# SludgePhD/Compeg

Hardware: AMD Instinct MI355X
Metric: Mpixels/s decoded (4K 4:2:2 restart-interval baseline JPEG -> RGBA8 in HBM) (higher is better)
Workload: dtype u32 bit-reader / i16 levels / f32 IDCT / u8 RGBA

## Files before the change

compeg_amd/csrc/kernels.hip:

```cpp
#include <hip/hip_runtime.h>

#include <algorithm>
#include <atomic>
#include <cstdio>
#include <cstdlib>

#include "kernels_body.h"
#include "coop_body.h"
#include "walk_body.h"
#include "kernels.h"
#include "lab.h"

namespace compeg {

struct DeviceLimits {
    uint32_t cus, lds_bytes;
};
static DeviceLimits device_limits()
{
    static std::atomic<uint64_t> known[64];
    int dev = 0;
    const bool indexed = hipGetDevice(&dev) == hipSuccess && dev >= 0 && dev < 64;
    if (indexed) {
        const uint64_t k = known[dev].load(std::memory_order_relaxed);
// ... 63 lines not shown
    const ImageDesc &d = descs[blockIdx.y];
    const uint32_t first_interval = blockIdx.x * blockDim.x;
    if (first_interval >= d.total_intervals)
        return;

    uint16_t *l1 = reinterpret_cast<uint16_t *>(smem);
    uint16_t *l2 = l1 + kL1Entries;
    const uint32_t wave_area = align16(window_words * 4u) + kWave * kDuSlotBytes;
    uint8_t *wave_base = smem + align16((kL1Entries + l2_in_lds) * 2u);

    stage_luts(d, l1, l2, l2_in_lds, threadIdx.x, blockDim.x);

    const uint32_t wave = threadIdx.x / kWave, lane = threadIdx.x % kWave;
    uint32_t *win = reinterpret_cast<uint32_t *>(wave_base + wave * wave_area);
    const uint32_t wave_first = first_interval + wave * kWave;
    uint32_t win_base = 0, win_len = 0;
    if (wave_first < d.total_intervals) {
        wave_window(d, wave_first, window_words, win_base, win_len);
        stage_window(d, win, win_base, win_len, lane);
    }
    __syncthreads();

    if (wave_first >= d.total_intervals)
        return;

    HuffShared s;
    s.l1 = l1;
    s.l2 = l2;
    s.l2_staged = umin(l2_in_lds, d.fast_off + 2u * kFastEntries);
    s.win = win;
    s.win_base = win_base;
    s.win_len = win_len;
    s.du_slots = reinterpret_cast<uint8_t *>(win) + align16(window_words * 4u);
    entropy_wave_to_records<SAMPLES>(d, s, wave_first + lane, lane);
}

__global__ void __launch_bounds__(1024)
entropy_kernel(const ImageDesc *__restrict__ descs, uint32_t l2_in_lds, uint32_t window_words)
{
    entropy_kernel_body<false>(descs, l2_in_lds, window_words);
}

__global__ void __launch_bounds__(768)
entropy_samples_kernel(const ImageDesc *__restrict__ descs, uint32_t l2_in_lds, uint32_t window_words)
{
    entropy_kernel_body<true>(descs, l2_in_lds, window_words);
}

struct WindowAhead {
    const ImageDesc *descs;
    uint32_t image;
    bool any;
    uint32_t first;
    uint32_t window_words, lane;
    uint32_t *win;
    uint32_t raw_base, raw_end, base, len, sink;
    uint32_t *queue;
    uint32_t next, drawn, stride, units, waves_per_image, group;

    __device__ __forceinline__ void at(uint32_t du, uint32_t du_total)
    {
        if (queue) {
            if (du == 0u && lane == 0u)
                drawn = atomicAdd(queue, 1u);
            if (du == 1u) {
                next = (stride + uint32_t(__builtin_amdgcn_readfirstlane(int(drawn)))) * group;
                any = next < units;
                if (any) {
                    image = uint32_t(__builtin_amdgcn_readfirstlane(int(next / waves_per_image)));
                    first = uint32_t(__builtin_amdgcn_readfirstlane(int((next % waves_per_image) * kWave)));
                }
            }
        }
        if (!any)
            return;
        const ImageDesc *dn = descs + image;
        if (du == (queue ? 1u : 0u))
            wave_window_fetch(*dn, first, raw_base, raw_end);
        if (du_total >= 8u && du == (du_total >= 10u ? du_total - 8u : 2u)) {
            uint32_t b, l;
            wave_window_from(*dn, raw_base, raw_end, window_words, b, l);
            const uint32_t have = dn->nwords > b ? umin(l, dn->nwords - b) : 0u;
            auto *words = CG_GLOBAL(const uint32_t, dn->words);
            for (uint32_t v = lane * 32u; v < have; v += kWave * 32u)
                sink ^= words[b + v];
        }
        if (du_total >= 8u && du == (du_total >= 10u ? du_total - 5u : 5u))
            asm volatile("" ::"v"(sink));
    }

    __device__ __forceinline__ void decoded(uint32_t du, uint32_t du_total)
    {
        if (!any || du + 1u != du_total)
            return;
        const ImageDesc *dn = descs + image;
        uint32_t b, l;
        wave_window_from(*dn, raw_base, raw_end, window_words, b, l);
        base = uint32_t(__builtin_amdgcn_readfirstlane(int(b)));
        len = uint32_t(__builtin_amdgcn_readfirstlane(int(l)));
        stage_window(*dn, win, base, len, lane);
        __builtin_amdgcn_fence(__ATOMIC_RELEASE, "wavefront");
        __builtin_amdgcn_wave_barrier();
    }
};

template <class LAYOUT, uint32_t GROUP>
__device__ __forceinline__ void fused_kernel_body(const ImageDesc *__restrict__ descs, uint32_t l2_in_lds, uint32_t window_words,
                                                  uint32_t waves_per_image, uint32_t images, uint32_t *queue)
{
    constexpr uint32_t group = GROUP;
    extern __shared__ __attribute__((aligned(16))) uint8_t smem[];
    const uint32_t wave = uint32_t(__builtin_amdgcn_readfirstlane(int(threadIdx.x / kWave))), lane = threadIdx.x % kWave;
    uint32_t image = blockIdx.y, wave_first = (blockIdx.x * (blockDim.x / kWave) + wave) * kWave;
    bool has_work = true;
    if (waves_per_image) {
        const uint32_t flat = (blockIdx.x * (blockDim.x / kWave) + wave) * (queue ? group : 1u);
        image = flat / waves_per_image;
        wave_first = (flat % waves_per_image) * kWave;
        has_work = image < images;
        image = has_work ? image : images - 1u;
    }
    image = uint32_t(__builtin_amdgcn_readfirstlane(int(image)));
    wave_first = uint32_t(__builtin_amdgcn_readfirstlane(int(wave_first)));
    if (!waves_per_image && blockIdx.x * blockDim.x >= descs[image].total_intervals)
        return;
    has_work = has_work && wave_first < descs[image].total_intervals;

    uint16_t *l1 = reinterpret_cast<uint16_t *>(smem);
    uint16_t *l2 = l1 + kL1Entries;
    const uint32_t wave_area = align16(window_words * 4u) + kWave * kDuSlotBytes;
    uint8_t *wave_base = smem + align16((kL1Entries + l2_in_lds) * 2u);
    uint32_t *win = reinterpret_cast<uint32_t *>(wave_base + wave * wave_area);
    uint8_t *slots = reinterpret_cast<uint8_t *>(win) + align16(window_words * 4u);

    uint32_t win_base = 0, win_len = 0;
    if (has_work)
        wave_window(descs[image], wave_first, window_words, win_base, win_len);
    stage_luts_and_window(descs[image], l1, l2, l2_in_lds, threadIdx.x, blockDim.x, win, win_base, win_len, lane);
    __syncthreads();

    if (!has_work)
        return;

    const uint32_t stride = gridDim.x * (blockDim.x / kWave), units = waves_per_image * images;
    const uint32_t per_draw = waves_per_image && queue ? group : 1u;
    uint32_t flat = (blockIdx.x * (blockDim.x / kWave) + wave) * per_draw;
    for (;;) {
        const ImageDesc &d = descs[image];
        HuffShared s;
        s.l1 = l1;
        s.l2 = l2;
        s.l2_staged = umin(l2_in_lds, d.fast_off + 2u * kFastEntries);
        s.win = win;
        s.win_base = win_base;
        s.win_len = win_len;
        s.du_slots = slots;
        const bool draw = waves_per_image && queue && flat % per_draw == per_draw - 1u;
        flat += waves_per_image && queue ? 1u : stride;
        WindowAhead ahead;
        ahead.descs = descs;
        ahead.queue = draw ? queue : nullptr;
        ahead.stride = stride;
        ahead.units = units;
        ahead.waves_per_image = waves_per_image;
        ahead.group = per_draw;
        ahead.next = ahead.drawn = 0u;
        ahead.any = waves_per_image && !draw && flat < units;
        ahead.image = ahead.first = 0u;
        if (ahead.any) {
            ahead.image = uint32_t(__builtin_amdgcn_readfirstlane(int(flat / waves_per_image)));
            ahead.first = uint32_t(__builtin_amdgcn_readfirstlane(int((flat % waves_per_image) * kWave)));
        }
        ahead.window_words = window_words;
        ahead.lane = lane;
        ahead.win = win;
        ahead.sink = 0u;
        LAYOUT::decode(d, s, wave_first + lane, lane, ahead);
        if (!ahead.any)
            break;
        if (draw)
            flat = ahead.next;
        image = ahead.image;
        wave_first = ahead.first;
        win_base = ahead.base;
        win_len = ahead.len;
    }
}

constexpr uint32_t kMcuQueueGroup = 4;

template <bool WIDE, bool RECORDS = false>
struct Wave422 {
    template <class AHEAD>
    static __device__ __forceinline__ void decode(const ImageDesc &d, const HuffShared &s, uint32_t interval, uint32_t lane, AHEAD &ahead)
    {
        decode_wave_fused_422<AHEAD, WIDE, RECORDS>(d, s, interval, lane, ahead);
    }
};
#if !defined(CG_FUSED_BOUNDS) || !defined(COMPEG_LAB)
#define CG_FUSED_BOUNDS 768
#endif
__global__ void __launch_bounds__(CG_FUSED_BOUNDS)
decode_fused_422_kernel(const ImageDesc *__restrict__ descs, uint32_t l2_in_lds, uint32_t window_words,
                        uint32_t waves_per_image, uint32_t images, uint32_t *queue)
{
    fused_kernel_body<Wave422<false>, 1>(descs, l2_in_lds, window_words, waves_per_image, images, queue);
}
__global__ void __launch_bounds__(768)
decode_fused_422_mcu_kernel(const ImageDesc *__restrict__ descs, uint32_t l2_in_lds, uint32_t window_words,
                            uint32_t waves_per_image, uint32_t images, uint32_t *queue)
{
    fused_kernel_body<Wave422<true>, kMcuQueueGroup>(descs, l2_in_lds, window_words, waves_per_image, images, queue);
}
__global__ void __launch_bounds__(768)
decode_fused_422_mcu_rec_kernel(const ImageDesc *__restrict__ descs, uint32_t l2_in_lds, uint32_t window_words,
                                uint32_t waves_per_image, uint32_t images, uint32_t *queue)
{
    fused_kernel_body<Wave422<true, true>, kMcuQueueGroup>(descs, l2_in_lds, window_words, waves_per_image, images, queue);
}
template <int HS, int VS, int MC>
__device__ __forceinline__ void fused_layout_kernel_body(const ImageDesc *__restrict__ descs, uint32_t l2_in_lds, uint32_t window_words)
{
    extern __shared__ __attribute__((aligned(16))) uint8_t smem[];
    const ImageDesc &d = descs[blockIdx.y];
    const uint32_t first_interval = blockIdx.x * blockDim.x;
    if (first_interval >= d.total_intervals)
        return;
    uint16_t *l1 = reinterpret_cast<uint16_t *>(smem);
    uint16_t *l2 = l1 + kL1Entries;
    const uint32_t wave_area = align16(window_words * 4u) + kWave * kDuSlotBytes;
    uint8_t *wave_base = smem + align16((kL1Entries + l2_in_lds) * 2u);
    const uint32_t wave = uint32_t(__builtin_amdgcn_readfirstlane(int(threadIdx.x / kWave))), lane = threadIdx.x % kWave;
    uint32_t *win = reinterpret_cast<uint32_t *>(wave_base + wave * wave_area);
    const uint32_t wave_first = first_interval + wave * kWave;
    uint32_t win_base = 0, win_len = 0;
    if (wave_first < d.total_intervals)
        wave_window(d, wave_first, window_words, win_base, win_len);
    stage_luts_and_window(d, l1, l2, l2_in_lds, threadIdx.x, blockDim.x, win, win_base, win_len, lane);
    __syncthreads();
    if (wave_first >= d.total_intervals)
        return;
// ... 1029 lines not shown
```

compeg_amd/csrc/kernels_body.h:

```cpp
#pragma once

#include <cstdint>
#include <cstring>

#include "device_types.h"

#if defined(__HIPCC__)
#define CG_DEV __device__ __forceinline__
#else
#define CG_DEV static inline
#endif

#if defined(__HIP_DEVICE_COMPILE__)
#define CG_GLOBAL(T, p) (reinterpret_cast<__attribute__((address_space(1))) T *>(reinterpret_cast<uintptr_t>(p)))
#define CG_PIN_SCALAR(x) asm volatile("" : "+s"(x))
#else
#define CG_GLOBAL(T, p) (p)
#define CG_PIN_SCALAR(x) (void)(x)
#endif

#ifndef CG_IDCT_PACKED
#define CG_IDCT_PACKED 1
#endif
#ifndef CG_PRIO_IDCT
#define CG_PRIO_IDCT 1
#endif
#ifndef CG_PRIO_ENTROPY
#define CG_PRIO_ENTROPY 0
#endif
#ifndef CG_PRIO_COMPOSITE
#define CG_PRIO_COMPOSITE 3
#endif
#ifndef CG_NT_STORES
#define CG_NT_STORES 1
#endif
#if !defined(COMPEG_LAB)
#undef CG_EXP
#endif
#ifndef CG_EXP
#define CG_EXP 0
#endif

namespace compeg {

struct alignas(16) Vec4u {
    uint32_t x, y, z, w;
};

template <bool STREAM>
CG_DEV void store_pixels(uint8_t *p, const Vec4u &v)
{
#if defined(COMPEG_LAB) && defined(CG_STORE_POLICY) && defined(__HIP_DEVICE_COMPILE__)
    if (STREAM) {
        typedef uint32_t u32x4 __attribute__((ext_vector_type(4)));
        const u32x4 val{v.x, v.y, v.z, v.w};
        asm volatile("global_store_dwordx4 %0, %1, off " CG_STORE_POLICY ::"v"(p), "v"(val) : "memory");
        return;
    }
#endif
#if CG_NT_STORES && defined(__HIP_DEVICE_COMPILE__)
    if (STREAM) {
        typedef uint32_t u32x4 __attribute__((ext_vector_type(4)));
        __builtin_nontemporal_store(
            u32x4{v.x, v.y, v.z, v.w},
            reinterpret_cast<__attribute__((address_space(1))) u32x4 *>(reinterpret_cast<uintptr_t>(p)));
        return;
    }
#endif
    *CG_GLOBAL(Vec4u, reinterpret_cast<Vec4u *>(p)) = v;
}


struct HuffShared {
    const uint16_t *l1;
    const uint16_t *l2;
    uint32_t l2_staged;
    const uint32_t *win;
    uint32_t win_base;
    uint32_t win_len;
    uint8_t *du_slots;
};

CG_DEV uint32_t bswap32(uint32_t w)
{
    return (w << 24) | ((w & 0xff00u) << 8) | ((w >> 8) & 0xff00u) | (w >> 24);
}

struct BitReader {
    uint32_t cur, nxt, left, next_word;
};

CG_DEV uint32_t fetch_word(const ImageDesc &d, const HuffShared &s, uint32_t idx)
{
    const uint32_t rel = idx - s.win_base;
    if (rel < s.win_len)
        return s.win[rel];
    return idx < d.nwords ? bswap32(CG_GLOBAL(const uint32_t, d.words)[idx]) : 0u;
}

CG_DEV void refill(BitReader &b, const ImageDesc &d, const HuffShared &s)
{
    if (b.left < 32u) {
        const uint32_t w = fetch_word(d, s, b.next_word);
        b.next_word += 1u;
        b.cur |= w >> (b.left & 31u);
        b.nxt = (w << 1) << ((31u - b.left) & 31u);
        b.left += 32u;
    }
}

CG_DEV void consume(BitReader &b, uint32_t n)
{
    b.cur = (b.cur << (n & 31u)) | ((b.nxt >> 1) >> ((31u - n) & 31u));
    b.nxt <<= (n & 31u);
    b.left -= n;
}

CG_DEV uint32_t peek(const BitReader &b, uint32_t n)
{
    return (b.cur >> 1) >> ((31u - n) & 31u);
}

CG_DEV int32_t huff_extend(int32_t v, uint32_t t)
// ... 947 lines not shown
    e.pred0 = comp == 0u ? p : p0;
    e.pred1 = comp == 1u ? p : p1;
    e.pred2 = comp == 2u ? p : p2;
    return int32_t(uint32_t(p) * d.dc_quant[comp]);
}


constexpr int kPxSlotWords = 17;

CG_DEV uint32_t ycbcr_to_rgba(uint32_t y_, uint32_t cb_, uint32_t cr_)
{
    const int32_t y = int32_t(y_), cb = int32_t(cb_) - 128, cr = int32_t(cr_) - 128;
    int32_t r = y + ((45 * cr) >> 5);
    int32_t g = y - ((11 * cb + 23 * cr) >> 5);
    int32_t b = y + ((113 * cb) >> 6);
    r = r < 0 ? 0 : (r > 255 ? 255 : r);
    g = g < 0 ? 0 : (g > 255 ? 255 : g);
    b = b < 0 ? 0 : (b > 255 ? 255 : b);
    return uint32_t(r) | uint32_t(g) << 8 | uint32_t(b) << 16 | 0xff000000u;
}

CG_DEV void composite_422(const ImageDesc &d, const uint32_t *px_slots, uint32_t first_mcu,
                          uint32_t total_mcus, uint32_t j)
{
    const uint32_t m = j >> 2, quarter = j & 3u;
    const uint32_t mcu = first_mcu + m;
    if (mcu >= total_mcus)
        return;
    const uint32_t mx = mcu % d.width_mcus, my = mcu / d.width_mcus;
    const uint32_t x0 = mx * 16u + quarter * 4u;
    if (x0 >= d.out_w)
        return;
    const uint32_t *ydu = px_slots + (m * 4u + (quarter >> 1)) * kPxSlotWords;
    const uint32_t *cbdu = px_slots + (m * 4u + 2u) * kPxSlotWords;
    const uint32_t *crdu = px_slots + (m * 4u + 3u) * kPxSlotWords;
    const uint32_t cshift = (quarter & 1u) * 16u;
#pragma unroll
    for (uint32_t row = 0; row < 8; row++) {
        const uint32_t y = my * 8u + row;
        if (y >= d.out_h)
            break;
        const uint32_t yw = ydu[row * 2u + (quarter & 1u)];
        const uint32_t cbw = cbdu[row * 2u + (quarter >> 1)] >> cshift;
        const uint32_t crw = crdu[row * 2u + (quarter >> 1)] >> cshift;
        Vec4u o;
        o.x = ycbcr_to_rgba(yw & 0xffu, cbw & 0xffu, crw & 0xffu);
        o.y = ycbcr_to_rgba((yw >> 8) & 0xffu, cbw & 0xffu, crw & 0xffu);
        o.z = ycbcr_to_rgba((yw >> 16) & 0xffu, (cbw >> 8) & 0xffu, (crw >> 8) & 0xffu);
        o.w = ycbcr_to_rgba(yw >> 24, (cbw >> 8) & 0xffu, (crw >> 8) & 0xffu);
        uint8_t *p = d.out + size_t(y) * d.out_pitch + size_t(x0) * 4u;
        if (x0 + 3u < d.out_w && (d.out_pitch & 15u) == 0u) {
            store_pixels<true>(p, o);
        } else {
            auto *q = CG_GLOBAL(uint32_t, reinterpret_cast<uint32_t *>(p));
            q[0] = o.x;
            if (x0 + 1u < d.out_w)
                q[1] = o.y;
            if (x0 + 2u < d.out_w)
                q[2] = o.z;
            if (x0 + 3u < d.out_w)
                q[3] = o.w;
        }
    }
}


CG_DEV uint32_t ycbcr_to_rgba(uint32_t y_, uint32_t cb_, uint32_t cr_);

CG_DEV Vec4u rgba_quad(uint32_t yw, uint32_t cb2, uint32_t cr2)
{
    Vec4u o;
#if defined(__HIP_DEVICE_COMPILE__)
    typedef short s2 __attribute__((ext_vector_type(2)));
    const s2 cb = __builtin_bit_cast(s2, __builtin_amdgcn_perm(0u, cb2, 0x0c010c00u));
    const s2 cr = __builtin_bit_cast(s2, __builtin_amdgcn_perm(0u, cr2, 0x0c010c00u));
    const s2 k45 = {45, 45}, k11 = {11, 11}, k23 = {23, 23}, k113 = {113, 113};
    const s2 b45 = {-5760, -5760}, b34 = {-4352, -4352}, b113 = {-14464, -14464};
    const s2 sh5 = {5, 5}, sh6 = {6, 6};
    const s2 rc = (cr * k45 + b45) >> sh5;
    const s2 gc = (cb * k11 + (cr * k23 + b34)) >> sh5;
    const s2 bc = (cb * k113 + b113) >> sh6;
    const s2 ya = __builtin_bit_cast(s2, yw & 0x00ff00ffu);
    const s2 yb = __builtin_bit_cast(s2, (yw >> 8) & 0x00ff00ffu);
    uint32_t ra, ga, ba, rb, gb, bb;
    asm("v_sat_pk_u8_i16 %0, %1" : "=v"(ra) : "v"(ya + rc));
    asm("v_sat_pk_u8_i16 %0, %1" : "=v"(ga) : "v"(ya - gc));
    asm("v_sat_pk_u8_i16 %0, %1" : "=v"(ba) : "v"(ya + bc));
    asm("v_sat_pk_u8_i16 %0, %1" : "=v"(rb) : "v"(yb + rc));
    asm("v_sat_pk_u8_i16 %0, %1" : "=v"(gb) : "v"(yb - gc));
    asm("v_sat_pk_u8_i16 %0, %1" : "=v"(bb) : "v"(yb + bc));
    const uint32_t rga = ga << 16 | ra, rgb = gb << 16 | rb;
    o.x = __builtin_amdgcn_perm(ba, rga, 0x0d040200u);
    o.z = __builtin_amdgcn_perm(ba, rga, 0x0d050301u);
    o.y = __builtin_amdgcn_perm(bb, rgb, 0x0d040200u);
    o.w = __builtin_amdgcn_perm(bb, rgb, 0x0d050301u);
#else
    o.x = ycbcr_to_rgba(yw & 0xffu, cb2 & 0xffu, cr2 & 0xffu);
    o.y = ycbcr_to_rgba((yw >> 8) & 0xffu, cb2 & 0xffu, cr2 & 0xffu);
    o.z = ycbcr_to_rgba((yw >> 16) & 0xffu, (cb2 >> 8) & 0xffu, (cr2 >> 8) & 0xffu);
    o.w = ycbcr_to_rgba(yw >> 24, (cb2 >> 8) & 0xffu, (cr2 >> 8) & 0xffu);
#endif
    return o;
}

CG_DEV Vec4u rgba_quad4(uint32_t yw, uint32_t cb4, uint32_t cr4)
{
    Vec4u o;
#if defined(__HIP_DEVICE_COMPILE__)
    typedef short s2 __attribute__((ext_vector_type(2)));
    const s2 k45 = {45, 45}, k11 = {11, 11}, k23 = {23, 23}, k113 = {113, 113};
    const s2 b45 = {-5760, -5760}, b34 = {-4352, -4352}, b113 = {-14464, -14464};
    const s2 sh5 = {5, 5}, sh6 = {6, 6};
    const s2 ya = __builtin_bit_cast(s2, yw & 0x00ff00ffu), yb = __builtin_bit_cast(s2, (yw >> 8) & 0x00ff00ffu);
    const s2 cba = __builtin_bit_cast(s2, cb4 & 0x00ff00ffu), cbb = __builtin_bit_cast(s2, (cb4 >> 8) & 0x00ff00ffu);
    const s2 cra = __builtin_bit_cast(s2, cr4 & 0x00ff00ffu), crb = __builtin_bit_cast(s2, (cr4 >> 8) & 0x00ff00ffu);
    uint32_t ra, ga, ba, rb, gb, bb;
    asm("v_sat_pk_u8_i16 %0, %1" : "=v"(ra) : "v"(ya + ((cra * k45 + b45) >> sh5)));
    asm("v_sat_pk_u8_i16 %0, %1" : "=v"(ga) : "v"(ya - ((cba * k11 + (cra * k23 + b34)) >> sh5)));
    asm("v_sat_pk_u8_i16 %0, %1" : "=v"(ba) : "v"(ya + ((cba * k113 + b113) >> sh6)));
    asm("v_sat_pk_u8_i16 %0, %1" : "=v"(rb) : "v"(yb + ((crb * k45 + b45) >> sh5)));
    asm("v_sat_pk_u8_i16 %0, %1" : "=v"(gb) : "v"(yb - ((cbb * k11 + (crb * k23 + b34)) >> sh5)));
    asm("v_sat_pk_u8_i16 %0, %1" : "=v"(bb) : "v"(yb + ((cbb * k113 + b113) >> sh6)));
    const uint32_t rga = ga << 16 | ra, rgb = gb << 16 | rb;
    o.x = __builtin_amdgcn_perm(ba, rga, 0x0d040200u);
    o.z = __builtin_amdgcn_perm(ba, rga, 0x0d050301u);
    o.y = __builtin_amdgcn_perm(bb, rgb, 0x0d040200u);
    o.w = __builtin_amdgcn_perm(bb, rgb, 0x0d050301u);
#else
    o.x = ycbcr_to_rgba(yw & 0xffu, cb4 & 0xffu, cr4 & 0xffu);
    o.y = ycbcr_to_rgba((yw >> 8) & 0xffu, (cb4 >> 8) & 0xffu, (cr4 >> 8) & 0xffu);
    o.z = ycbcr_to_rgba((yw >> 16) & 0xffu, (cb4 >> 16) & 0xffu, (cr4 >> 16) & 0xffu);
    o.w = ycbcr_to_rgba(yw >> 24, cb4 >> 24, cr4 >> 24);
#endif
    return o;
}


CG_DEV void composite_row_to_slot(const uint32_t (&px)[4][16], uint32_t row, uint8_t *slot)
{
    SlotVec *p = reinterpret_cast<SlotVec *>(slot);
#pragma unroll
    for (uint32_t q = 0; q < 4; q++) {
#if CG_EXP == 5
        p[q] = SlotVec{px[q >> 1][row * 2u + (q & 1u)], px[2][row * 2u + (q >> 1)], px[3][row * 2u + (q >> 1)], q};
#else
        const Vec4u o = rgba_quad(px[q >> 1][row * 2u + (q & 1u)], px[2][row * 2u + (q >> 1)] >> ((q & 1u) * 16u),
                                  px[3][row * 2u + (q >> 1)] >> ((q & 1u) * 16u));
        p[q] = SlotVec{o.x, o.y, o.z, o.w};
#endif
    }
}

CG_DEV void composite_row_from_quad(const ImageDesc &d, const uint8_t *wave_slots, uint32_t lane, uint32_t row,
                                    uint8_t *const (&bases)[4], uint32_t whole_mask)
{
    const uint32_t quad = lane & ~3u, piece = lane & 3u;
#pragma unroll
    for (uint32_t j = 0; j < 4; j++) {
        const SlotVec v = reinterpret_cast<const SlotVec *>(wave_slots + (quad + j) * kDuSlotBytes)[piece];
#if (CG_EXP == 9 || CG_EXP == 17 || CG_EXP == 18) && defined(__HIP_DEVICE_COMPILE__)
        asm volatile("" ::"v"(v.x), "v"(v.y), "v"(v.z), "v"(v.w));
        if (v.x == 0x12345678u && v.y == 0x9abcdef0u && bases[j] == nullptr)
#else
        if (whole_mask >> j & 1u)
#endif
        {
            store_pixels<true>(bases[j] + size_t(row) * d.out_pitch + piece * 16u, Vec4u{v.x, v.y, v.z, v.w});
        }
    }
}

CG_DEV uint32_t cut_rows_for_piece(uint32_t limits, uint32_t piece)
{
    uint32_t rows = 0u;
#pragma unroll
    for (uint32_t j = 0; j < 4; j++) {
        const uint32_t lim = (limits >> (8u * j)) & 0xffu;
        rows |= (piece < lim >> 5 ? lim & 31u : 0u) << (8u * j);
    }
    return rows;
}
CG_DEV uint32_t cut_row_inside(uint32_t rows, uint32_t row) { return (rows + 0x01010101u * (127u - row)) & 0x80808080u; }

CG_DEV void composite_row_from_wave(const ImageDesc &d, const uint8_t *wave_slots, uint32_t lane, uint32_t row,
                                    uint8_t *const (&bases)[4], uint32_t whole_mask)
{
    const uint32_t piece = lane & 3u, sub = lane >> 2;
#pragma unroll
    for (uint32_t t = 0; t < 4; t++) {
        const SlotVec v = reinterpret_cast<const SlotVec *>(wave_slots + (16u * t + sub) * kDuSlotBytes)[piece];
        if (whole_mask >> t & 1u)
            store_pixels<true>(bases[t] + size_t(row) * d.out_pitch + piece * 16u, Vec4u{v.x, v.y, v.z, v.w});
    }
}

CG_DEV void composite_edge_mcu(const ImageDesc &d, const uint32_t (&px)[4][16], uint32_t mx, uint32_t my)
{
    const uint32_t x0 = mx * 16u, y0 = my * 8u;
    uint8_t *base = d.out + size_t(y0) * d.out_pitch + size_t(x0) * 4u;
#pragma unroll 1
    for (uint32_t row = 0; row < 8; row++) {
        if (y0 + row >= d.out_h)
            break;
#pragma unroll 1
        for (uint32_t q = 0; q < 4; q++) {
            const uint32_t w = row * 2u + (q & 1u), c = row * 2u + (q >> 1);
            uint32_t yw = 0, cbw = 0, crw = 0;
#pragma unroll
            for (uint32_t i = 0; i < 16; i++) {
                yw = (i == w) ? ((q >> 1) ? px[1][i] : px[0][i]) : yw;
                cbw = (i == c) ? px[2][i] : cbw;
                crw = (i == c) ? px[3][i] : crw;
            }
            const Vec4u o = rgba_quad(yw, cbw >> ((q & 1u) * 16u), crw >> ((q & 1u) * 16u));
            const uint32_t x = x0 + q * 4u;
            auto *p = CG_GLOBAL(uint32_t, reinterpret_cast<uint32_t *>(base + size_t(row) * d.out_pitch + q * 16u));
            if (x < d.out_w)
                p[0] = o.x;
            if (x + 1u < d.out_w)
                p[1] = o.y;
            if (x + 2u < d.out_w)
                p[2] = o.z;
            if (x + 3u < d.out_w)
                p[3] = o.w;
        }
    }
}


CG_DEV void records_flush_quad(const ImageDesc &d, const uint8_t *wave_slots, uint32_t lane, uint32_t interval,
                               uint32_t du_in_interval, int32_t dc)
{
    const uint32_t quad = lane & ~3u, piece = lane & 3u;
    const uint32_t du_count = d.restart_interval * d.dus_per_mcu;
#pragma unroll
    for (uint32_t j = 0; j < 4; j++) {
        const uint32_t other = interval - piece + j;
        if (other < d.total_intervals) {
            const SlotVec v = reinterpret_cast<const SlotVec *>(wave_slots + (quad + j) * kDuSlotBytes)[piece];
            auto *rec = CG_GLOBAL(Vec4u, reinterpret_cast<Vec4u *>(
                                             d.ac + (size_t(other) * du_count + du_in_interval) * kRetained));
            rec[piece] = Vec4u{v.x, v.y, v.z, v.w};
        }
    }
    if (interval < d.total_intervals)
        CG_GLOBAL(int32_t, d.dc)[size_t(interval) * du_count + du_in_interval] = dc;
}

CG_DEV void slot_to_samples(const ImageDesc &d, uint32_t comp, uint8_t *slot, int32_t dc)
{
    uint32_t rec[kRetained / 2];
    take_slot(slot, rec);
    uint32_t px[16];
    idct_data_unit(rec, dc, d.quant[comp], px);
    SlotVec *p = reinterpret_cast<SlotVec *>(slot);
#pragma unroll
    for (int i = 0; i < 4; i++)
        p[i] = SlotVec{px[4 * i], px[4 * i + 1], px[4 * i + 2], px[4 * i + 3]};
}

#if defined(__HIPCC__)
template <bool SAMPLES>
CG_DEV void entropy_wave_to_records(const ImageDesc &d, const HuffShared &s, uint32_t interval, uint32_t lane)
{
    uint8_t *slot = s.du_slots + lane * kDuSlotBytes;
    int16_t *slot16 = reinterpret_cast<int16_t *>(slot);
    zero_slot(slot);

    EntropyState e;
    entropy_init(e, d, s, interval < d.total_intervals ? interval : d.total_intervals - 1u);

    const uint32_t dpm = d.dus_per_mcu;
    const uint32_t du_count = d.restart_interval * dpm;
    uint32_t k = 0;
#pragma unroll 1
    for (uint32_t du = 0; du < du_count; du++) {
        const uint32_t comp = (d.comp_of_du >> (2u * k)) & 3u;
        const int32_t dc = entropy_data_unit(e, d, s, comp < 3u ? comp : 2u, slot16);
        if (SAMPLES)
            slot_to_samples(d, comp < 3u ? comp : 2u, slot, dc);
        records_flush_quad(d, s.du_slots, lane, interval, du, dc);
        zero_slot(slot);
        k = k + 1u == dpm ? 0u : k + 1u;
    }
}
#endif


CG_DEV void composite_generic_4px(const ImageDesc &d, uint32_t x0, uint32_t y, const uint8_t *samples_, uint32_t mcu0)
{
    if (x0 >= d.out_w || y >= d.out_h)
        return;
    const uint32_t wsh = d.mcu_w == 16u ? 4u : 3u, hsh = d.mcu_h == 16u ? 4u : 3u;
    const uint32_t mcu_x = x0 >> wsh, mcu_y = y >> hsh;
    const uint32_t mcu = mcu_y * d.width_mcus + mcu_x;
    if (mcu_x >= d.width_mcus || mcu >= d.total_intervals * d.restart_interval)
        return;
    const uint32_t col = x0 & (d.mcu_w - 1u), row = y & (d.mcu_h - 1u);
    struct alignas(8) Row8 {
        uint32_t lo, hi;
    };
    const Row8 *samples = reinterpret_cast<const Row8 *>(samples_);
    uint32_t val[3];
#pragma unroll
    for (uint32_t c = 0; c < 3; c++) {
        const uint32_t hs = d.hsample[c], vs = d.vsample[c];
        const uint32_t xsh = (wsh - 3u) - (hs - 1u), ysh = (hsh - 3u) - (vs - 1u);
        const uint32_t yy = (row >> ysh) & 7u;
        const uint32_t du = d.du_base[c] + ((row * vs) >> hsh) * hs + ((col * hs) >> wsh);
        const Row8 r = samples[(size_t(mcu - mcu0) * d.dus_per_mcu + du) * 8u + yy];
        const uint64_t bits = uint64_t(r.hi) << 32 | r.lo;
        if (xsh == 0u) {
            val[c] = uint32_t(bits >> ((col & 7u) * 8u));
        } else {
            const uint32_t two = uint32_t(bits >> (((col >> 1) & 7u) * 8u));
            val[c] = (two & 0xffu) * 0x0101u | ((two >> 8) & 0xffu) * 0x01010000u;
        }
    }
    const Vec4u o = rgba_quad4(val[0], val[1], val[2]);
    uint8_t *p = d.out + size_t(y) * d.out_pitch + size_t(x0) * 4u;
    if (x0 + 3u < d.out_w && (d.out_pitch & 15u) == 0u) {
        store_pixels<true>(p, o);
        return;
    }
    auto *q = CG_GLOBAL(uint32_t, reinterpret_cast<uint32_t *>(p));
    q[0] = o.x;
    if (x0 + 1u < d.out_w)
        q[1] = o.y;
    if (x0 + 2u < d.out_w)
        q[2] = o.z;
    if (x0 + 3u < d.out_w)
        q[3] = o.w;
}

struct PixelState {
    uint32_t px[4][16];
    uint32_t mx, my;
    bool active;
};

CG_DEV void pixel_init(PixelState &t, const ImageDesc &d, uint32_t interval, bool active)
{
#pragma unroll
    for (int k = 0; k < 4; k++)
#pragma unroll
        for (int w = 0; w < 16; w++)
            t.px[k][w] = 0u;
    const uint32_t mcu = interval * d.restart_interval;
    t.mx = mcu % d.width_mcus;
    t.my = mcu / d.width_mcus;
    t.active = active;
}

#if defined(__HIP_DEVICE_COMPILE__)
#define CG_PLACE_MARK(text) asm volatile(text)
#else
#define CG_PLACE_MARK(text) do { } while (0)
#endif

CG_DEV void pixel_transform(PixelState &t, const ImageDesc &d, uint32_t comp, uint32_t k, uint8_t *slot, int32_t dc)
{
    uint32_t rec[kRetained / 2];
    take_slot(slot, rec);
#if CG_EXP == 4 || CG_EXP == 17
#pragma unroll
    for (int w = 0; w < 16; w++)
        t.px[3][w] = rec[w] + uint32_t(dc);
#elif CG_EXP == 16 || CG_EXP == 18
    if (k >= 2u) {
#pragma unroll
        for (int w = 0; w < 16; w++)
            t.px[3][w] = rec[w] + uint32_t(dc);
    } else {
        idct_data_unit(rec, dc, d.quant[comp], t.px[3]);
    }
#else
    idct_data_unit(rec, dc, d.quant[comp], t.px[3]);
#endif
    if (k == 0u) {
#pragma unroll
        for (int w = 0; w < 16; w++)
            t.px[0][w] = t.px[3][w];
        CG_PLACE_MARK("; data unit 0 in place");
    } else if (k == 1u) {
#pragma unroll
        for (int w = 0; w < 16; w++)
            t.px[1][w] = t.px[3][w];
        CG_PLACE_MARK("; data unit 1 in place");
    } else if (k == 2u) {
#pragma unroll
        for (int w = 0; w < 16; w++)
            t.px[2][w] = t.px[3][w];
        CG_PLACE_MARK("; data unit 2 in place");
    }
}

struct McuTarget {
    uint8_t *base;
    bool whole;
};

CG_DEV uint32_t target_limit(const ImageDesc &d, bool active, uint32_t x0, uint32_t y0, uint32_t w, uint32_t h)
{
    const uint32_t px_in = x0 < d.out_w ? umin(w, d.out_w - x0) : 0u, rows_in = y0 < d.out_h ? umin(h, d.out_h - y0) : 0u;
    return active && (d.out_pitch & 15u) == 0u && (px_in & 3u) == 0u && px_in && rows_in ? rows_in | (px_in >> 2) << 5 : 0u;
}

CG_DEV McuTarget mcu_target(const PixelState &t, const ImageDesc &d)
{
#if CG_EXP == 14
    const uint32_t mcu = t.my * d.width_mcus + t.mx, unit = mcu & ~255u, lane_ = (mcu >> 2) & 63u, m_ = mcu & 3u;
    const uint32_t moved = umin(unit + 64u * (lane_ & 3u) + 16u * m_ + (lane_ >> 2), d.total_intervals * d.restart_interval - 1u);
    const uint32_t x0 = (moved % d.width_mcus) * 16u, y0 = (moved / d.width_mcus) * 8u;
#else
    const uint32_t x0 = t.mx * 16u, y0 = t.my * 8u;
#endif
    McuTarget g;
    g.base = d.out + size_t(y0) * d.out_pitch + size_t(x0) * 4u;
    g.whole = t.active && x0 + 16u <= umax(d.out_w, d.out_pitch / 4u) && y0 + 8u <= umax(d.out_h, d.out_alloc_h) && (d.out_pitch & 15u) == 0u &&
              x0 < d.out_w && y0 < d.out_h;
    return g;
}

CG_DEV void pixel_next_mcu(PixelState &t, const ImageDesc &d)
{
    t.mx++;
    if (t.mx == d.width_mcus) {
        t.mx = 0;
        t.my++;
    }
}

CG_DEV bool wave_any(bool v)
{
#if defined(__HIP_DEVICE_COMPILE__)
    return __builtin_amdgcn_ballot_w64(v) != 0u;
#else
    return v;
#endif
}


#if defined(COMPEG_LAB) && defined(CG_STREAM_LDSDMA) && defined(__HIP_DEVICE_COMPILE__)
#define CG_GLDS_ROW(J) \
    "global_load_lds_dword %[voff], %[base] offset:" #J "*256\n\t" \
    "s_cmp_eq_u32 %[n], " #J "+1\n\t" \
    "s_cbranch_scc1 9f\n\t" \
    "v_add_u32 %[voff], 0xffffff04, %[voff]\n\t"
#endif

#if defined(__HIP_DEVICE_COMPILE__)
typedef uint32_t QuadWordsAligned __attribute__((ext_vector_type(4)));
typedef QuadWordsAligned QuadWords __attribute__((aligned(4)));
#endif

CG_DEV void stream_stage_rows(const ImageDesc &d, uint32_t *rows, uint32_t nrows, uint32_t first, uint32_t lane)
{
#if defined(COMPEG_LAB) && defined(CG_STREAM_LDSDMA) && defined(__HIP_DEVICE_COMPILE__)
    (void)lane;
#if defined(CG_LDSDMA_TRY) && (CG_LDSDMA_TRY & 4)
    asm volatile("s_waitcnt vmcnt(0)" ::: "memory");
#else
    asm volatile("s_waitcnt vmcnt(40)" ::: "memory");
#endif
#if defined(CG_LDSDMA_TRY) && (CG_LDSDMA_TRY & 8)
    asm volatile("s_waitcnt lgkmcnt(0)" ::: "memory");
#endif
#if defined(CG_LDSDMA_TRY) && (CG_LDSDMA_TRY & 2)
    uint32_t keep_m0;
    asm volatile("s_mov_b32 %0, m0" : "=s"(keep_m0)::"memory");
#endif
    const uint8_t *base = reinterpret_cast<const uint8_t *>(d.words) - 4096;
    uint32_t m0 = uint32_t(reinterpret_cast<uintptr_t>(rows));
#pragma unroll 1
    for (uint32_t j = 0; j < nrows; j += 16u) {
        uint32_t voff = (first + j) * 4u + 4096u, n = umin(16u, nrows - j);
        if (j)
            asm volatile("s_waitcnt vmcnt(0)" ::: "memory");
        asm volatile("s_mov_b32 m0, %[m0]\n\t"
                     "s_nop 0\n\t"
                     CG_GLDS_ROW(0) CG_GLDS_ROW(1) CG_GLDS_ROW(2) CG_GLDS_ROW(3) CG_GLDS_ROW(4) CG_GLDS_ROW(5) CG_GLDS_ROW(6)
                         CG_GLDS_ROW(7) CG_GLDS_ROW(8) CG_GLDS_ROW(9) CG_GLDS_ROW(10) CG_GLDS_ROW(11) CG_GLDS_ROW(12)
                             CG_GLDS_ROW(13) CG_GLDS_ROW(14) CG_GLDS_ROW(15) "9:"
                     : [voff] "+v"(voff)
                     : [m0] "s"(m0), [base] "s"(base), [n] "s"(n)
                     : "memory", "scc");
        m0 += 16u * uint32_t(kWave) * 4u;
    }
#if defined(CG_LDSDMA_TRY) && (CG_LDSDMA_TRY & 2)
    asm volatile("s_mov_b32 m0, %0" ::"s"(keep_m0) : "memory");
#endif
#elif defined(__HIP_DEVICE_COMPILE__) && !defined(CG_STAGE_DWORDS)
    auto *words = CG_GLOBAL(const uint32_t, d.words);
    const uint32_t whole = nrows & ~3u;
#pragma unroll 4
    for (uint32_t j = 0; j < whole; j += 4u) {
        const QuadWords q = *reinterpret_cast<const __attribute__((address_space(1))) QuadWords *>(words + first + j);
        CG_LDS(uint32_t, rows)[(j + 0u) * uint32_t(kWave) + lane] = q.x;
        CG_LDS(uint32_t, rows)[(j + 1u) * uint32_t(kWave) + lane] = q.y;
        CG_LDS(uint32_t, rows)[(j + 2u) * uint32_t(kWave) + lane] = q.z;
        CG_LDS(uint32_t, rows)[(j + 3u) * uint32_t(kWave) + lane] = q.w;
    }
    for (uint32_t j = whole; j < nrows; j++)
        CG_LDS(uint32_t, rows)[j * uint32_t(kWave) + lane] = words[first + j];
#elif defined(__HIP_DEVICE_COMPILE__)
    auto *words = CG_GLOBAL(const uint32_t, d.words);
#pragma unroll 8
    for (uint32_t j = 0; j < nrows; j++)
        CG_LDS(uint32_t, rows)[j * uint32_t(kWave) + lane] = words[first + j];
#else
    for (uint32_t j = 0; j < nrows; j++)
        rows[j * uint32_t(kWave) + lane] = first + j < d.nwords ? d.words[first + j] : 0xfeedf00du;
// ... 32 lines not shown
    }
    e.resume = false;
}

CG_DEV bool stream_wants_rows(const EntropyState &e, const ImageDesc &d, const HuffShared &s, uint32_t lane, uint32_t below)
{
    if (!e.fast)
        return e.resume && e.r.left < 64u;
    const uint32_t left = uint32_t(e.wlimit - e.wptr) / uint32_t(kWave);
    const uint32_t end_word = e.r.next_word + uint32_t(e.wlimit - (s.win + lane)) / uint32_t(kWave);
    return left < below && end_word < d.nwords;
}

CG_DEV void stream_lane_init(EntropyState &e, const ImageDesc &d, const HuffShared &s, uint32_t nrows, uint32_t interval, uint32_t lane)
{
    reader_init(e.r, d, s, interval < d.nstarts ? CG_GLOBAL(const uint32_t, d.starts)[interval] : 0u);
    reader_refill<false>(e.r, d, s);
    e.pred0 = e.pred1 = e.pred2 = 0;
    e.ref_left = 32u;
    e.fast = false;
    e.resume = fast_tables_usable(d, s);
    e.wptr = e.wlimit = s.win + lane;
    stream_restage(e, d, s, nrows, lane);
}


CG_DEV void entropy_init_from_record(EntropyState &e, const ImageDesc &d, const HuffShared &s, uint32_t mcu)
{
    const uint32_t word = mcu < d.nstarts ? CG_GLOBAL(const uint32_t, d.starts)[mcu] : 0u;
    const McuState st = CG_GLOBAL(const McuState, d.mcu_state)[mcu];
    const uint32_t bit = st.info & 31u, left = (st.info >> 5) & 63u;
    e.pred0 = st.pred[0];
    e.pred1 = st.pred[1];
    e.pred2 = st.pred[2];
    e.wlimit = nullptr;
    e.resume = false;
    if (st.info & kMcuDead) {
        e.r.buf = 0u;
        e.r.left = 0xffffff00u;
        e.r.next_word = word;
        e.r.pre = 0u;
        e.ref_left = 0u;
        e.fast = false;
        e.wptr = s.win;
        return;
    }
    const bool two = bit + left > 32u;
    const uint32_t w0 = fetch_word_pf<false>(d, s, word), w1 = two ? fetch_word_pf<false>(d, s, word + 1u) : 0u;
    e.r.buf = (uint64_t(w0) << 32 | w1) << bit;
    e.r.left = left;
    e.r.next_word = word + (two ? 2u : 1u);
    e.r.pre = fetch_word_pf<false>(d, s, e.r.next_word);
    e.ref_left = left;
    const uint32_t rel = e.r.next_word - s.win_base;
    e.fast = fast_tables_usable(d, s) && rel < s.win_len;
    e.wptr = s.win + (e.fast ? rel : 0u);
}

#if defined(__HIPCC__)
template <int J>
CG_DEV uint32_t quad_lane(uint32_t v)
{
#if defined(__HIP_DEVICE_COMPILE__)
    return uint32_t(__builtin_amdgcn_update_dpp(0, int(v), J * 0x55, 0xf, 0xf, true));
#else
    return v;
#endif
}

template <int T>
CG_DEV uint32_t wave_lane(uint32_t v, uint32_t lane)
{
#if defined(__HIP_DEVICE_COMPILE__)
    return uint32_t(__builtin_amdgcn_ds_bpermute(int((16u * T + (lane >> 2)) * 4u), int(v)));
#else
    (void)lane;
    return v;
#endif
}

template <bool QUADS, bool WIDE = false>
CG_DEV void composite_mcus_422(PixelState &t, const ImageDesc &d, uint8_t *wave_slots, uint32_t lane)
{
    const McuTarget g = mcu_target(t, d);
    if (!QUADS) {
        if (g.whole) {
#pragma unroll
            for (uint32_t row = 0; row < 8; row++) {
#pragma unroll
                for (uint32_t q = 0; q < 4; q++)
                    store_pixels<false>(g.base + size_t(row) * d.out_pitch + q * 16u,
                                 rgba_quad(t.px[q >> 1][row * 2u + (q & 1u)], t.px[2][row * 2u + (q >> 1)] >> ((q & 1u) * 16u),
                                           t.px[3][row * 2u + (q >> 1)] >> ((q & 1u) * 16u)));
            }
        } else if (t.active) {
            composite_edge_mcu(d, t.px, t.mx, t.my);
        }
        pixel_next_mcu(t, d);
        return;
    }
    const uint64_t addr = reinterpret_cast<uint64_t>(g.base);
    const uint32_t lo = uint32_t(addr), hi = uint32_t(addr >> 32), wh = g.whole ? 1u : 0u;
    uint8_t *slot = wave_slots + lane * kDuSlotBytes;
    if (WIDE) {
        uint8_t *from[4] = {
            reinterpret_cast<uint8_t *>(uint64_t(wave_lane<0>(hi, lane)) << 32 | wave_lane<0>(lo, lane)),
            reinterpret_cast<uint8_t *>(uint64_t(wave_lane<1>(hi, lane)) << 32 | wave_lane<1>(lo, lane)),
            reinterpret_cast<uint8_t *>(uint64_t(wave_lane<2>(hi, lane)) << 32 | wave_lane<2>(lo, lane)),
            reinterpret_cast<uint8_t *>(uint64_t(wave_lane<3>(hi, lane)) << 32 | wave_lane<3>(lo, lane)),
        };
        const uint32_t mask = wave_lane<0>(wh, lane) | wave_lane<1>(wh, lane) << 1 | wave_lane<2>(wh, lane) << 2 | wave_lane<3>(wh, lane) << 3;
        if (__builtin_amdgcn_ballot_w64(mask != 0xfu) == 0u) {
#pragma unroll
            for (uint32_t row = 0; row < 8; row++) {
                composite_row_to_slot(t.px, row, slot);
                composite_row_from_wave(d, wave_slots, lane, row, from, 0xfu);
                __builtin_amdgcn_sched_barrier(0);
            }
        } else {
#pragma unroll
            for (uint32_t row = 0; row < 8; row++) {
                composite_row_to_slot(t.px, row, slot);
                composite_row_from_wave(d, wave_slots, lane, row, from, mask);
                __builtin_amdgcn_sched_barrier(0);
            }
        }
        zero_slot(slot);
        if (t.active && !g.whole)
            composite_edge_mcu(d, t.px, t.mx, t.my);
        pixel_next_mcu(t, d);
        return;
    }
    uint8_t *bases[4] = {
        reinterpret_cast<uint8_t *>(uint64_t(quad_lane<0>(hi)) << 32 | quad_lane<0>(lo)),
        reinterpret_cast<uint8_t *>(uint64_t(quad_lane<1>(hi)) << 32 | quad_lane<1>(lo)),
        reinterpret_cast<uint8_t *>(uint64_t(quad_lane<2>(hi)) << 32 | quad_lane<2>(lo)),
        reinterpret_cast<uint8_t *>(uint64_t(quad_lane<3>(hi)) << 32 | quad_lane<3>(lo)),
    };
    const uint32_t whole_mask = quad_lane<0>(wh) | quad_lane<1>(wh) << 1 | quad_lane<2>(wh) << 2 | quad_lane<3>(wh) << 3;
#if CG_EXP == 15
    if (__builtin_amdgcn_ballot_w64(whole_mask != 0xfu) == 0u) {
        uint8_t *left[4] = {bases[0] - 64, bases[1] - 64, bases[2] - 64, bases[3] - 64};
#pragma unroll
        for (uint32_t row = 0; row < 8; row++) {
            composite_row_to_slot(t.px, row, slot);
            if (t.mx & 1u) {
                composite_row_from_quad(d, wave_slots, lane, row, left, 0xfu);
                composite_row_from_quad(d, wave_slots, lane, row, bases, 0xfu);
            }
            __builtin_amdgcn_sched_barrier(0);
        }
    } else
#endif
    if (__builtin_amdgcn_ballot_w64(whole_mask != 0xfu) == 0u) {
#pragma unroll
        for (uint32_t row = 0; row < 8; row++) {
            composite_row_to_slot(t.px, row, slot);
            composite_row_from_quad(d, wave_slots, lane, row, bases, 0xfu);
            __builtin_amdgcn_sched_barrier(0);
        }
    } else {
#pragma unroll
        for (uint32_t row = 0; row < 8; row++) {
            composite_row_to_slot(t.px, row, slot);
            composite_row_from_quad(d, wave_slots, lane, row, bases, whole_mask);
            __builtin_amdgcn_sched_barrier(0);
        }
    }
    zero_slot(slot);
    if (t.active && !g.whole)
        composite_edge_mcu(d, t.px, t.mx, t.my);
    pixel_next_mcu(t, d);
}

struct NothingAhead {
    CG_DEV void at(uint32_t, uint32_t) {}
    CG_DEV void decoded(uint32_t, uint32_t) {}
};

template <class AHEAD, bool WIDE = false, bool RECORDS = false>
CG_DEV void decode_wave_fused_422(const ImageDesc &d, const HuffShared &s, uint32_t interval, uint32_t lane, AHEAD &ahead)
{
    const bool active = interval < d.total_intervals;
    interval = active ? interval : d.total_intervals - 1u;
    uint8_t *slot = s.du_slots + lane * kDuSlotBytes;
    int16_t *slot16 = reinterpret_cast<int16_t *>(slot);
    zero_slot(slot);

    EntropyState e;
    PixelState t;
    if (RECORDS)
        entropy_init_from_record(e, d, s, interval);
    else
        entropy_init(e, d, s, interval);
    pixel_init(t, d, interval, active);
    __builtin_amdgcn_s_setprio(CG_PRIO_ENTROPY);

#if defined(CG_STAMPS) && defined(__HIP_DEVICE_COMPILE__)
#define CG_STAMP(acc) do { const uint64_t now_ = __builtin_readcyclecounter(); acc += now_ - tprev; tprev = now_; } while (0)
    uint64_t tprev = __builtin_readcyclecounter(), t_dc = 0, t_ac = 0, t_idct = 0, t_comp = 0;
#else
#define CG_STAMP(acc) do { } while (0)
#endif
    const uint32_t du_total = d.restart_interval * 4u;
#pragma unroll 1
    for (uint32_t du = 0; du < du_total; du++) {
        const uint32_t k = du & 3u;
        const uint32_t comp = k < 2u ? 0u : k - 1u;
        ahead.at(du, du_total);
        const int32_t dc = entropy_data_unit(e, d, s, comp, slot16);
        CG_STAMP(t_ac);
        ahead.decoded(du, du_total);
        __builtin_amdgcn_s_setprio(CG_PRIO_IDCT);
        pixel_transform(t, d, comp, k, slot, dc);
        CG_STAMP(t_idct);
        if (k == 3u) {
            __builtin_amdgcn_s_setprio(CG_PRIO_COMPOSITE);
            composite_mcus_422<true, WIDE>(t, d, s.du_slots, lane);
            CG_STAMP(t_comp);
        }
        __builtin_amdgcn_s_setprio(CG_PRIO_ENTROPY);
    }
#if defined(CG_STAMPS) && defined(__HIP_DEVICE_COMPILE__)
    if (lane == 0 && d.dc) {
        uint64_t *o = reinterpret_cast<uint64_t *>(d.dc) + size_t(interval / 64u) * 4u;
        o[0] = t_dc;
        o[1] = t_ac;
        o[2] = t_idct;
        o[3] = t_comp;
    }
#endif
}

CG_DEV void decode_wave_fused_422(const ImageDesc &d, const HuffShared &s, uint32_t interval, uint32_t lane)
{
    NothingAhead none;
    decode_wave_fused_422(d, s, interval, lane, none);
}

CG_DEV void decode_wave_fused_422_stream(const ImageDesc &d, const HuffShared &s, uint32_t nrows, uint32_t stage_after, uint32_t stage_below,
                                         uint32_t interval, uint32_t lane)
{
    const bool active = interval < d.total_intervals;
    interval = active ? interval : d.total_intervals - 1u;
    uint8_t *slot = s.du_slots + lane * kDuSlotBytes;
    int16_t *slot16 = reinterpret_cast<int16_t *>(slot);
    zero_slot(slot);

    EntropyState e;
    PixelState t;
    stream_lane_init(e, d, s, nrows, interval, lane);
    pixel_init(t, d, interval, active);
    stream_rows_landed();
    __builtin_amdgcn_s_setprio(CG_PRIO_ENTROPY);

    const uint32_t du_total = d.restart_interval * 4u;
#pragma unroll 1
    for (uint32_t du = 0; du < du_total; du++) {
        const uint32_t k = du & 3u;
        const uint32_t comp = k < 2u ? 0u : k - 1u;
        const int32_t dc = entropy_data_unit<true>(e, d, s, comp, slot16, lane);
        bool stage = ((stage_after | 8u) >> k & 1u) != 0u && du + 1u < du_total;
        if (stage)
            stage = wave_any(stream_wants_rows(e, d, s, lane, stage_below));
        if (stage)
            stream_restage(e, d, s, nrows, lane);
        __builtin_amdgcn_s_setprio(CG_PRIO_IDCT);
        pixel_transform(t, d, comp, k, slot, dc);
        if (stage)
            stream_rows_landed();
        if (k == 3u) {
            __builtin_amdgcn_s_setprio(CG_PRIO_COMPOSITE);
            composite_mcus_422<true>(t, d, s.du_slots, lane);
        }
        __builtin_amdgcn_s_setprio(CG_PRIO_ENTROPY);
    }
}

#endif

template <int HS, int VS, int MC>
struct LayoutPixels {
    static constexpr int kDus = HS * VS + 2;
    uint32_t px[MC * kDus][16];
    uint32_t mx, my;
    bool active;
};

template <int HS, int VS, int MC>
CG_DEV Vec4u layout_pixels4(const LayoutPixels<HS, VS, MC> &t, int row, int g)
{
    constexpr int kDus = HS * VS + 2;
    const int m = g / (2 * HS), gg = g % (2 * HS), o = m * kDus;
    const uint32_t yw = t.px[o + (row >> 3) * HS + (gg >> 1)][(row & 7) * 2 + (gg & 1)];
    const int cy = row / VS;
    if (HS == 2)
        return rgba_quad(yw, t.px[o + kDus - 2][cy * 2 + (gg >> 1)] >> ((gg & 1) * 16), t.px[o + kDus - 1][cy * 2 + (gg >> 1)] >> ((gg & 1) * 16));
    return rgba_quad4(yw, t.px[o + kDus - 2][cy * 2 + gg], t.px[o + kDus - 1][cy * 2 + gg]);
}

template <int HS, int VS, int MC>
// ... 324 lines not shown
```

Baseline: 768,400.

## Use 32-bit output offsets for near outputs and fuse packed saturations

When the output buffer fits in 4 GiB, the composite stage now swizzles 32-bit per-MCU offsets across lanes instead of 64-bit base pointers, cutting cross-lane moves and VGPR use. The YCbCr conversion merges the R and G saturations into one register with an SDWA word write, which drops the shift-or packing. It also pins the prefetch lane and the loop counter into scalar registers, and adds an optional workgroup store-turn throttle that only compiles in lab builds. The inline SDWA asm and the extra offset bookkeeping add risk of encoding or edge-case errors.

```diff
diff --git a/compeg_amd/csrc/kernels.hip b/compeg_amd/csrc/kernels.hip
--- a/compeg_amd/csrc/kernels.hip
+++ b/compeg_amd/csrc/kernels.hip
@@ -169,7 +169,9 @@
             wave_window_from(*dn, raw_base, raw_end, window_words, b, l);
             const uint32_t have = dn->nwords > b ? umin(l, dn->nwords - b) : 0u;
             auto *words = CG_GLOBAL(const uint32_t, dn->words);
-            for (uint32_t v = lane * 32u; v < have; v += kWave * 32u)
+            uint32_t ln = lane;
+            asm volatile("" : "+v"(ln));
+            for (uint32_t v = ln * 32u; v < have; v += kWave * 32u)
                 sink ^= words[b + v];
         }
         if (du_total >= 8u && du == (du_total >= 10u ? du_total - 5u : 5u))
@@ -224,6 +226,7 @@
     if (has_work)
         wave_window(descs[image], wave_first, window_words, win_base, win_len);
     stage_luts_and_window(descs[image], l1, l2, l2_in_lds, threadIdx.x, blockDim.x, win, win_base, win_len, lane);
+    store_turn_reset(threadIdx.x);
     __syncthreads();
 
     if (!has_work)
@@ -244,6 +247,7 @@
         s.du_slots = slots;
         const bool draw = waves_per_image && queue && flat % per_draw == per_draw - 1u;
         flat += waves_per_image && queue ? 1u : stride;
+        flat = uint32_t(__builtin_amdgcn_readfirstlane(int(flat)));
         WindowAhead ahead;
         ahead.descs = descs;
         ahead.queue = draw ? queue : nullptr;
diff --git a/compeg_amd/csrc/kernels_body.h b/compeg_amd/csrc/kernels_body.h
--- a/compeg_amd/csrc/kernels_body.h
+++ b/compeg_amd/csrc/kernels_body.h
@@ -39,6 +39,18 @@
 #endif
 #ifndef CG_EXP
 #define CG_EXP 0
+#endif
+#if !defined(COMPEG_LAB)
+#undef CG_TURNS
+#endif
+#ifndef CG_TURNS
+#define CG_TURNS 0
+#endif
+#ifndef CG_TURN_POLLS
+#define CG_TURN_POLLS 64
+#endif
+#ifndef CG_TURN_SLEEP
+#define CG_TURN_SLEEP 2
 #endif
 
 namespace compeg {
@@ -1152,14 +1164,15 @@
     const s2 bc = (cb * k113 + b113) >> sh6;
     const s2 ya = __builtin_bit_cast(s2, yw & 0x00ff00ffu);
     const s2 yb = __builtin_bit_cast(s2, (yw >> 8) & 0x00ff00ffu);
-    uint32_t ra, ga, ba, rb, gb, bb;
-    asm("v_sat_pk_u8_i16 %0, %1" : "=v"(ra) : "v"(ya + rc));
-    asm("v_sat_pk_u8_i16 %0, %1" : "=v"(ga) : "v"(ya - gc));
-    asm("v_sat_pk_u8_i16 %0, %1" : "=v"(ba) : "v"(ya + bc));
-    asm("v_sat_pk_u8_i16 %0, %1" : "=v"(rb) : "v"(yb + rc));
-    asm("v_sat_pk_u8_i16 %0, %1" : "=v"(gb) : "v"(yb - gc));
-    asm("v_sat_pk_u8_i16 %0, %1" : "=v"(bb) : "v"(yb + bc));
-    const uint32_t rga = ga << 16 | ra, rgb = gb << 16 | rb;
+    uint32_t rga, ba, rgb, bb;
+    asm("v_sat_pk_u8_i16 %0, %1" : "=v"(rga) : "v"(ya + rc));
+    asm("v_sat_pk_u8_i16_sdwa %0, %2 dst_sel:WORD_1 dst_unused:UNUSED_PRESERVE src0_sel:DWORD\n\tv_sat_pk_u8_i16 %1, %3"
+        : "+v"(rga), "=v"(ba)
+        : "v"(ya - gc), "v"(ya + bc));
+    asm("v_sat_pk_u8_i16 %0, %1" : "=v"(rgb) : "v"(yb + rc));
+    asm("v_sat_pk_u8_i16_sdwa %0, %2 dst_sel:WORD_1 dst_unused:UNUSED_PRESERVE src0_sel:DWORD\n\tv_sat_pk_u8_i16 %1, %3"
+        : "+v"(rgb), "=v"(bb)
+        : "v"(yb - gc), "v"(yb + bc));
     o.x = __builtin_amdgcn_perm(ba, rga, 0x0d040200u);
     o.z = __builtin_amdgcn_perm(ba, rga, 0x0d050301u);
     o.y = __builtin_amdgcn_perm(bb, rgb, 0x0d040200u);
@@ -1240,6 +1253,18 @@
     }
 }
 
+CG_DEV void composite_row_from_quad_near(uint8_t *row_base, const uint8_t *wave_slots, uint32_t lane, const uint32_t (&offs)[4],
+                                         uint32_t whole_mask)
+{
+    const uint32_t quad = lane & ~3u, piece = lane & 3u;
+#pragma unroll
+    for (uint32_t j = 0; j < 4; j++) {
+        const SlotVec v = reinterpret_cast<const SlotVec *>(wave_slots + (quad + j) * kDuSlotBytes)[piece];
+        if (whole_mask >> j & 1u)
+            store_pixels<true>(row_base + size_t(offs[j]), Vec4u{v.x, v.y, v.z, v.w});
+    }
+}
+
 CG_DEV uint32_t cut_rows_for_piece(uint32_t limits, uint32_t piece)
 {
     uint32_t rows = 0u;
@@ -1261,6 +1286,17 @@
         const SlotVec v = reinterpret_cast<const SlotVec *>(wave_slots + (16u * t + sub) * kDuSlotBytes)[piece];
         if (whole_mask >> t & 1u)
             store_pixels<true>(bases[t] + size_t(row) * d.out_pitch + piece * 16u, Vec4u{v.x, v.y, v.z, v.w});
+    }
+}
+CG_DEV void composite_row_from_wave_near(uint8_t *row_base, const uint8_t *wave_slots, uint32_t lane, const uint32_t (&offs)[4],
+                                         uint32_t whole_mask)
+{
+    const uint32_t piece = lane & 3u, sub = lane >> 2;
+#pragma unroll
+    for (uint32_t t = 0; t < 4; t++) {
+        const SlotVec v = reinterpret_cast<const SlotVec *>(wave_slots + (16u * t + sub) * kDuSlotBytes)[piece];
+        if (whole_mask >> t & 1u)
+            store_pixels<true>(row_base + size_t(offs[t]), Vec4u{v.x, v.y, v.z, v.w});
     }
 }
 
@@ -1406,6 +1442,7 @@
 struct PixelState {
     uint32_t px[4][16];
     uint32_t mx, my;
+    uint32_t off;
     bool active;
 };
 
@@ -1419,6 +1456,7 @@
     const uint32_t mcu = interval * d.restart_interval;
     t.mx = mcu % d.width_mcus;
     t.my = mcu / d.width_mcus;
+    t.off = t.my * 8u * d.out_pitch + t.mx * 64u;
     t.active = active;
 }
 
@@ -1492,12 +1530,27 @@
     return g;
 }
 
+CG_DEV bool output_near(const ImageDesc &d)
+{
+#if CG_EXP == 14 || CG_EXP == 15
+    return false;
+#else
+    uint32_t far_ = uint32_t((uint64_t(d.out_pitch) * umax(d.out_h, d.out_alloc_h)) >> 32);
+#if defined(__HIP_DEVICE_COMPILE__)
+    far_ = uint32_t(__builtin_amdgcn_readfirstlane(int(far_)));
+#endif
+    return far_ == 0u;
+#endif
+}
+
 CG_DEV void pixel_next_mcu(PixelState &t, const ImageDesc &d)
 {
     t.mx++;
+    t.off += 64u;
     if (t.mx == d.width_mcus) {
         t.mx = 0;
         t.my++;
+        t.off += 8u * d.out_pitch - 64u * d.width_mcus;
     }
 }
 
@@ -1696,6 +1749,7 @@
 template <bool QUADS, bool WIDE = false>
 CG_DEV void composite_mcus_422(PixelState &t, const ImageDesc &d, uint8_t *wave_slots, uint32_t lane)
 {
+    const bool near = QUADS && output_near(d);
     const McuTarget g = mcu_target(t, d);
     if (!QUADS) {
         if (g.whole) {
@@ -1713,9 +1767,57 @@
         pixel_next_mcu(t, d);
         return;
     }
+    const uint32_t wh = g.whole ? 1u : 0u;
+    uint8_t *slot = wave_slots + lane * kDuSlotBytes;
+    if (near) {
+        const uint32_t piece16 = (lane & 3u) * 16u;
+        if (WIDE) {
+            const uint32_t offs[4] = {wave_lane<0>(t.off, lane) + piece16, wave_lane<1>(t.off, lane) + piece16,
+                                      wave_lane<2>(t.off, lane) + piece16, wave_lane<3>(t.off, lane) + piece16};
+            const uint32_t mask = wave_lane<0>(wh, lane) | wave_lane<1>(wh, lane) << 1 | wave_lane<2>(wh, lane) << 2 | wave_lane<3>(wh, lane) << 3;
+            if (__builtin_amdgcn_ballot_w64(mask != 0xfu) == 0u) {
+#pragma unroll
+                for (uint32_t row = 0; row < 8; row++) {
+                    composite_row_to_slot(t.px, row, slot);
+                    composite_row_from_wave_near(d.out + size_t(row) * d.out_pitch, wave_slots, lane, offs, 0xfu);
+                    __builtin_amdgcn_sched_barrier(0);
+                }
+            } else {
+#pragma unroll
+                for (uint32_t row = 0; row < 8; row++) {
+                    composite_row_to_slot(t.px, row, slot);
+                    composite_row_from_wave_near(d.out + size_t(row) * d.out_pitch, wave_slots, lane, offs, mask);
+                    __builtin_amdgcn_sched_barrier(0);
+                }
+            }
+        } else {
+            const uint32_t offs[4] = {quad_lane<0>(t.off) + piece16, quad_lane<1>(t.off) + piece16, quad_lane<2>(t.off) + piece16,
+                                      quad_lane<3>(t.off) + piece16};
+            const uint32_t whole_mask = quad_lane<0>(wh) | quad_lane<1>(wh) << 1 | quad_lane<2>(wh) << 2 | quad_lane<3>(wh) << 3;
+            if (__builtin_amdgcn_ballot_w64(whole_mask != 0xfu) == 0u) {
+#pragma unroll
+                for (uint32_t row = 0; row < 8; row++) {
+                    composite_row_to_slot(t.px, row, slot);
+                    composite_row_from_quad_near(d.out + size_t(row) * d.out_pitch, wave_slots, lane, offs, 0xfu);
+                    __builtin_amdgcn_sched_barrier(0);
+                }
+            } else {
+#pragma unroll
+                for (uint32_t row = 0; row < 8; row++) {
+                    composite_row_to_slot(t.px, row, slot);
+                    composite_row_from_quad_near(d.out + size_t(row) * d.out_pitch, wave_slots, lane, offs, whole_mask);
+                    __builtin_amdgcn_sched_barrier(0);
+                }
+            }
+        }
+        zero_slot(slot);
+        if (t.active && !g.whole)
+            composite_edge_mcu(d, t.px, t.mx, t.my);
+        pixel_next_mcu(t, d);
+        return;
+    }
     const uint64_t addr = reinterpret_cast<uint64_t>(g.base);
-    const uint32_t lo = uint32_t(addr), hi = uint32_t(addr >> 32), wh = g.whole ? 1u : 0u;
-    uint8_t *slot = wave_slots + lane * kDuSlotBytes;
+    const uint32_t lo = uint32_t(addr), hi = uint32_t(addr >> 32);
     if (WIDE) {
         uint8_t *from[4] = {
             reinterpret_cast<uint8_t *>(uint64_t(wave_lane<0>(hi, lane)) << 32 | wave_lane<0>(lo, lane)),
@@ -1786,6 +1888,45 @@
         composite_edge_mcu(d, t.px, t.mx, t.my);
     pixel_next_mcu(t, d);
 }
+
+#if CG_TURNS > 0 && defined(__HIP_DEVICE_COMPILE__)
+CG_DEV uint32_t *store_turn_counter()
+{
+    __shared__ uint32_t storing;
+    return &storing;
+}
+CG_DEV void store_turn_enter(uint32_t lane)
+{
+    uint32_t *n = store_turn_counter();
+    __builtin_amdgcn_s_setprio(CG_PRIO_ENTROPY);
+#pragma unroll 1
+    for (uint32_t poll = 0;; poll++) {
+        uint32_t before = 0u;
+        if (lane == 0u)
+            before = __hip_atomic_fetch_add(n, 1u, __ATOMIC_RELAXED, __HIP_MEMORY_SCOPE_WORKGROUP);
+        before = uint32_t(__builtin_amdgcn_readfirstlane(int(before)));
+        if (before < uint32_t(CG_TURNS) || poll >= uint32_t(CG_TURN_POLLS))
+            return;
+        if (lane == 0u)
+            __hip_atomic_fetch_sub(n, 1u, __ATOMIC_RELAXED, __HIP_MEMORY_SCOPE_WORKGROUP);
+        __builtin_amdgcn_s_sleep(CG_TURN_SLEEP);
+    }
+}
+CG_DEV void store_turn_leave(uint32_t lane)
+{
+    if (lane == 0u)
+        __hip_atomic_fetch_sub(store_turn_counter(), 1u, __ATOMIC_RELAXED, __HIP_MEMORY_SCOPE_WORKGROUP);
+}
+CG_DEV void store_turn_reset(uint32_t thread)
+{
+    if (thread == 0u)
+        *store_turn_counter() = 0u;
+}
+#else
+CG_DEV void store_turn_enter(uint32_t) {}
+CG_DEV void store_turn_leave(uint32_t) {}
+CG_DEV void store_turn_reset(uint32_t) {}
+#endif
 
 struct NothingAhead {
     CG_DEV void at(uint32_t, uint32_t) {}
@@ -1829,8 +1970,10 @@
         pixel_transform(t, d, comp, k, slot, dc);
         CG_STAMP(t_idct);
         if (k == 3u) {
+            store_turn_enter(lane);
             __builtin_amdgcn_s_setprio(CG_PRIO_COMPOSITE);
             composite_mcus_422<true, WIDE>(t, d, s.du_slots, lane);
+            store_turn_leave(lane);
             CG_STAMP(t_comp);
         }
         __builtin_amdgcn_s_setprio(CG_PRIO_ENTROPY);
```

Measured after the change: 778,200, median of 6. Within noise of the previous version (+1.3%).
